# GenkiK/monodepth2

Measured on AMD Instinct MI355X. Metric: training images/sec at 640x192 mono, 1/2/4/8 GPUs; loss delta vs ref, higher is better.
Workload: dtype f32; 1 GPU; mono_640x192 ResNet-18 batch=12/GPU full train step (configs[1]); global_batch=12, height=192, width=640, parallelism=dp1, step=hipgraph replay

## Files before the change

### include/md2hot.h

```cpp
#ifndef MD2HOT_H
#define MD2HOT_H

#include <stddef.h>
#include <stdint.h>

#ifdef __cplusplus
extern "C" {
#endif

#define MD2_ABI_VERSION 24
#define MD2_MAX_SCALES 4
#define MD2_MAX_SRC 3

#define MD2_OK 0
#define MD2_ERR_ARG (-1)
#define MD2_ERR_HIP (-2)

#define MD2_NO_SSIM          (1u << 0)
#define MD2_AVG_REPROJECTION (1u << 1)
#define MD2_NO_AUTOMASK      (1u << 2)
#define MD2_V1_MULTISCALE    (1u << 3)
#define MD2_T_PER_SCALE      (1u << 4)
#define MD2_PREDICTIVE_MASK  (1u << 5)

// ... 66 lines not shown
size_t md2_decoder_pad_workspace_bytes(const md2_pad_desc* desc);
int md2_decoder_pad_fwd(const md2_pad_desc* desc, const float* x, const float* skip, const float* bias,
                        float* out, void* stream);
int md2_decoder_pad_bwd(const md2_pad_desc* desc, const float* x, const float* bias, const float* grad_out,
                        float* grad_x, float* grad_skip, float* grad_bias, void* workspace, void* stream);
int md2_decoder_pad_bwd2(const md2_pad_desc* desc, const float* x, const float* bias, const float* grad_out,
                         const float* grad_out2, float* grad_x, float* grad_skip, float* grad_bias, void* workspace,
                         void* stream);

#define MD2_HEAD_WEIGHT_CL (1u << 0)
#define MD2_HEAD_BF16 (1u << 1)

typedef struct md2_head_desc {
    int32_t batch, channels, height, width;
    uint32_t flags;
} md2_head_desc;

size_t md2_disp_head_workspace_bytes(const md2_head_desc* desc);
int md2_disp_head_fwd(const md2_head_desc* desc, const float* padded, const float* weight, const float* bias,
                      float* disp, void* stream);
int md2_disp_head_bwd(const md2_head_desc* desc, const float* padded, const float* weight, const float* disp,
                      const float* grad_disp, float* grad_padded, float* grad_weight, float* grad_bias,
                      void* workspace, void* stream);

#define MD2_STEM_WEIGHT_CL (1u << 0)
#define MD2_STEM_BF16 (1u << 1)
#define MD2_STEM_PREFETCH (1u << 2)

typedef struct md2_stem_desc {
    int32_t batch, channels, height, width;
    uint32_t flags;
} md2_stem_desc;

size_t md2_stem_wgrad_workspace_bytes(const md2_stem_desc* desc);
int md2_stem_wgrad(const md2_stem_desc* desc, const float* x, const float* grad_y, float* grad_weight,
                   void* workspace, void* stream);

int md2_stem_fwd(const md2_stem_desc* desc, const float* x, const float* weight, float* y, void* stream);

#define MD2_BIAS_ACT_RELU (1u << 0)

typedef struct md2_bias_act_desc {
    int64_t pixels;
    int32_t channels;
    uint32_t flags;
} md2_bias_act_desc;
// ... 266 lines not shown
```

### monodepth2_amd/_lib.py

```python
from __future__ import annotations

import ctypes
import os
import threading

import torch

from .build import LIB_PATH as _BUILT_LIB
from .build import source_hash

LIB_PATH = os.environ.get("MD2_LIB", _BUILT_LIB)

MAX_SCALES = 4
MAX_SRC = 3
ABI_VERSION = 24

NO_SSIM = 1 << 0
AVG_REPROJECTION = 1 << 1
NO_AUTOMASK = 1 << 2
V1_MULTISCALE = 1 << 3
T_PER_SCALE = 1 << 4
PREDICTIVE_MASK = 1 << 5

_vp = ctypes.c_void_p
# ... 23 lines not shown
_lib = None

EXPORTS = ["md2_abi_version", "md2_last_error", "md2_workspace_bytes", "md2_select_bytes",
           "md2_photometric_fwd", "md2_photometric_bwd", "md2_generate_images", "md2_tiebreak_noise",
           "md2_timing_begin", "md2_timing_end", "md2_timing_calls", "md2_decoder_pad_fwd", "md2_decoder_pad_bwd",
           "md2_decoder_pad_workspace_bytes", "md2_adam_step", "md2_adam_step_dev", "md2_adam_hyper", "md2_adam_apply_dev", "md2_encoder_input",
           "md2_pose_fwd", "md2_pose_bwd", "md2_aug_plan_create", "md2_aug_plan_destroy", "md2_aug_run",
           "md2_bn_workspace_bytes", "md2_bn_fwd", "md2_bn_bwd", "md2_maxpool3s2_fwd", "md2_maxpool3s2_bwd",
           "md2_disp_head_workspace_bytes", "md2_disp_head_fwd", "md2_disp_head_bwd",
           "md2_stem_wgrad_workspace_bytes", "md2_stem_wgrad", "md2_stem_fwd", "md2_conv_col2im", "md2_bias_act_fwd", "md2_bias_act_bwd",
           "md2_bias_act_workspace_bytes", "md2_maxpool3s2_bwd_add", "md2_bn_bwd_multi",
           "md2_conv_fwd", "md2_conv_workspace_bytes", "md2_conv_split_weights",
           "md2_conv_dgrad", "md2_conv_wgrad", "md2_conv_direct", "md2_conv_wgrad_direct",
           "md2_conv_wgrad_direct_workspace_bytes", "md2_conv_split_weights_multi", "md2_bn_fwd_mask",
           "md2_bn_bwd_mask", "md2_build_id", "md2_maxpool3s2_bwd_multi", "md2_decoder_pad_bwd2", "md2_aug_run2",
           "md2_conv_bf16_weights", "md2_conv_bf16_weights_multi",
           "md2_depth_eval", "md2_depth_eval_workspace_bytes",
           "md2_velo_project", "md2_velo_project_workspace_bytes",
           "md2_pose_ate", "md2_pose_ate_workspace_bytes",
           "md2_disp_colorize", "md2_disp_colorize_workspace_bytes",
           "md2_bn_pool_fwd_supported", "md2_bn_pool_fwd", "md2_bn_bwd_reduce_mask", "md2_bn_coef_offset",
           "md2_stem_wgrad_bn_supported", "md2_stem_wgrad_bn",
           "md2_aug_plan_create_mixed", "md2_aug_run_mixed",
           "md2_depth_export16", "md2_depth_export16_check"]

DTYPE_F32 = 0
DTYPE_BF16 = 1
PAD_ELU = 1 << 0
PAD_UPSAMPLE = 1 << 1
PAD_NHWC = 1 << 2
PAD_BF16 = 1 << 3


class PadDesc(ctypes.Structure):
    _fields_ = [("batch", ctypes.c_int32), ("channels", ctypes.c_int32), ("height", ctypes.c_int32),
                ("width", ctypes.c_int32), ("skip_channels", ctypes.c_int32), ("flags", ctypes.c_uint32)]


class AugDesc(ctypes.Structure):
    _fields_ = [("items", ctypes.c_int32), ("frames", ctypes.c_int32), ("in_height", ctypes.c_int32),
                ("in_width", ctypes.c_int32), ("height", ctypes.c_int32), ("width", ctypes.c_int32),
                ("num_scales", ctypes.c_int32), ("reserved", ctypes.c_int32)]


class AugItem(ctypes.Structure):
    _fields_ = [("flip", ctypes.c_uint8), ("color_aug", ctypes.c_uint8), ("hue_shift", ctypes.c_uint8),
                ("reserved", ctypes.c_uint8), ("order", ctypes.c_uint8 * 4), ("brightness", ctypes.c_float),
# ... 173 lines not shown
    L.md2_conv_split_weights.argtypes = [ctypes.POINTER(ConvDesc)] + [_vp] * 4
    L.md2_conv_split_weights_multi.restype = ctypes.c_int
    L.md2_conv_split_weights_multi.argtypes = [_vp, ctypes.c_int, ctypes.c_int, _vp]
    L.md2_conv_bf16_weights.restype = ctypes.c_int
    L.md2_conv_bf16_weights.argtypes = [ctypes.POINTER(ConvDesc)] + [_vp] * 4
    L.md2_conv_bf16_weights_multi.restype = ctypes.c_int
    L.md2_conv_bf16_weights_multi.argtypes = [_vp, ctypes.c_int, ctypes.c_int, _vp]
    L.md2_conv_workspace_bytes.restype = ctypes.c_size_t
    L.md2_conv_workspace_bytes.argtypes = [ctypes.POINTER(ConvDesc)]
    L.md2_stem_wgrad_workspace_bytes.restype = ctypes.c_size_t
    L.md2_stem_wgrad_workspace_bytes.argtypes = [ctypes.POINTER(StemDesc)]
    L.md2_stem_wgrad.restype = ctypes.c_int
    L.md2_stem_wgrad.argtypes = [ctypes.POINTER(StemDesc)] + [_vp] * 5
    L.md2_stem_fwd.restype = ctypes.c_int
    L.md2_conv_col2im.restype = ctypes.c_int
    L.md2_conv_col2im.argtypes = [ctypes.POINTER(ConvDesc)] + [_vp] * 3
    L.md2_stem_fwd.argtypes = [ctypes.POINTER(StemDesc)] + [_vp] * 4
    L.md2_disp_head_workspace_bytes.restype = ctypes.c_size_t
    L.md2_disp_head_workspace_bytes.argtypes = [ctypes.POINTER(HeadDesc)]
    L.md2_disp_head_fwd.restype = ctypes.c_int
    L.md2_disp_head_fwd.argtypes = [ctypes.POINTER(HeadDesc)] + [_vp] * 5
    L.md2_disp_head_bwd.restype = ctypes.c_int
    L.md2_disp_head_bwd.argtypes = [ctypes.POINTER(HeadDesc)] + [_vp] * 9
    L.md2_abi_version.restype = ctypes.c_int
    L.md2_abi_version.argtypes = []
    L.md2_build_id.restype = ctypes.c_char_p
    L.md2_build_id.argtypes = []
    L.md2_last_error.restype = ctypes.c_char_p
    L.md2_last_error.argtypes = []
    L.md2_workspace_bytes.restype = ctypes.c_size_t
    L.md2_workspace_bytes.argtypes = [ctypes.POINTER(Desc)]
    L.md2_select_bytes.restype = ctypes.c_size_t
    L.md2_select_bytes.argtypes = [ctypes.POINTER(Desc)]
    L.md2_photometric_fwd.restype = ctypes.c_int
    L.md2_photometric_fwd.argtypes = [ctypes.POINTER(Desc), ctypes.POINTER(Tensors), _vp, _vp, _vp, _vp]
    L.md2_photometric_bwd.restype = ctypes.c_int
    L.md2_photometric_bwd.argtypes = [ctypes.POINTER(Desc), ctypes.POINTER(Tensors), _vp, _vp,
                                      ctypes.POINTER(_vp), _vp, _vp, _vp, _vp]
    L.md2_generate_images.restype = ctypes.c_int
    L.md2_generate_images.argtypes = [ctypes.POINTER(Desc), ctypes.POINTER(Tensors),
                                      ctypes.POINTER(_vp), ctypes.POINTER(_vp), ctypes.POINTER(_vp), _vp]
    L.md2_tiebreak_noise.restype = ctypes.c_int
    L.md2_tiebreak_noise.argtypes = [ctypes.POINTER(Desc), _vp, ctypes.c_int, _vp, _vp]
    L.md2_decoder_pad_fwd.restype = ctypes.c_int
    L.md2_decoder_pad_fwd.argtypes = [ctypes.POINTER(PadDesc), _vp, _vp, _vp, _vp, _vp]
    L.md2_decoder_pad_bwd.restype = ctypes.c_int
# ... 125 lines not shown
```

### monodepth2_amd/build.py

```python
from __future__ import annotations

import hashlib
import os
import shutil
import subprocess
import sys

HERE = os.path.dirname(os.path.abspath(__file__))
CSRC = os.path.join(HERE, "csrc")
INCLUDE = os.path.join(os.path.dirname(HERE), "include")
LIB_NAME = "libmd2hot.so"
LIB_PATH = os.path.join(CSRC, LIB_NAME)
SOURCES = ["md2hot.hip", "decoder.hip", "pose.hip", "augment.hip", "bnorm.hip", "pool.hip", "adam.hip", "disphead.hip", "stem.hip", "bias_act.hip", "conv.hip", "direct.hip", "glue.hip", "eval.hip", "velo.hip", "traj.hip", "viz.hip"]
HEADERS = [os.path.join(INCLUDE, "md2hot.h"), os.path.join(CSRC, "md2_bf16.h"), os.path.join(CSRC, "md2_bn_expr.h"),
           os.path.join(CSRC, "md2_x6.h")]
ARCH = os.environ.get("MD2_OFFLOAD_ARCH", "gfx950")


def hipcc() -> str:
    for cand in (os.environ.get("HIPCC"), "/opt/rocm/bin/hipcc", shutil.which("hipcc")):
        if cand and os.path.exists(cand):
            return cand
    raise RuntimeError("hipcc not found (ROCm toolchain required to build libmd2hot.so)")


def needs_build() -> bool:
    if not os.path.exists(LIB_PATH):
        return True
    t = os.path.getmtime(LIB_PATH)
    deps = [os.path.join(CSRC, s) for s in SOURCES] + HEADERS
    if any(os.path.getmtime(d) > t for d in deps):
        return True
    return built_id(LIB_PATH) != source_hash()


def built_id(path: str):
    try:
        with open(path, "rb") as f:
# ... 62 lines not shown
```

### monodepth2_amd/csrc/decoder.hip

```cpp

#include <hip/hip_runtime.h>

#include <stdint.h>
#include <stdlib.h>

#include "md2_bf16.h"
#include "md2hot.h"

namespace {

constexpr int kThreads = 256;

__device__ __forceinline__ int reflect1(int i, int n) {
    return i < 0 ? -i : (i >= n ? 2 * n - 2 - i : i);
}

__device__ __forceinline__ float elu(float v) { return v > 0.f ? v : expm1f(v); }
__device__ __forceinline__ float elu_grad(float v) { return v > 0.f ? 1.f : expm1f(v) + 1.f; }

struct PadArgs {
    int B, C, Cs, h, w, H, W;
    const float* x;
    const float* skip;
    float* out;
    const float* gout;
    const float* gout2;
    float* gx;
    float* gskip;
    const float* bias;
    float* gbias_part;
};

template <bool NHWC>
__device__ __forceinline__ size_t at(int b, int c, int y, int x, int C, int Hh, int Ww) {
    return NHWC ? (((size_t)b * Hh + y) * Ww + x) * C + c : (((size_t)b * C + c) * Hh + y) * Ww + x;
}

template <bool ELU, bool UP, bool NHWC>
__global__ __launch_bounds__(kThreads) void pad_fwd_kernel(PadArgs a) {
    const int Hp = a.H + 2, Wp = a.W + 2, Ct = a.C + a.Cs;
    const long long total = (long long)a.B * Ct * Hp * Wp;
    for (long long idx = (long long)blockIdx.x * kThreads + threadIdx.x; idx < total;
         idx += (long long)gridDim.x * kThreads) {
        int px, py, c, b;
        long long t;
        if (NHWC) {
            c = (int)(idx % Ct);
            t = idx / Ct;
            px = (int)(t % Wp);
            t /= Wp;
            py = (int)(t % Hp);
            b = (int)(t / Hp);
        } else {
// ... 66 lines not shown
        int b, c, i, j;
        if (idx < nx) {
            coords<NHWC>(idx, a.C, a.h, a.w, b, c, i, j);
            const float* g = a.gout + at<NHWC>(b, c, 0, 0, Ct, Hp, Wp);
            float s;
            if (UP) {
                s = fold(g, Wp, a.H, a.W, 2 * i, 2 * j, es) + fold(g, Wp, a.H, a.W, 2 * i, 2 * j + 1, es) +
                    fold(g, Wp, a.H, a.W, 2 * i + 1, 2 * j, es) + fold(g, Wp, a.H, a.W, 2 * i + 1, 2 * j + 1, es);
            } else {
                s = fold(g, Wp, a.H, a.W, i, j, es);
            }
            if (ELU) s *= elu_grad(a.x[idx]);
            a.gx[idx] = s;
        } else {
            const long long k = idx - nx;
            coords<NHWC>(k, a.Cs, a.H, a.W, b, c, i, j);
            a.gskip[k] = fold(a.gout + at<NHWC>(b, a.C + c, 0, 0, Ct, Hp, Wp), Wp, a.H, a.W, i, j, es);
        }
    }
}

__device__ __forceinline__ float4 ld4(const float* p) { return *(const float4*)p; }
__device__ __forceinline__ void st4(float* p, float4 v) { *(float4*)p = v; }
__device__ __forceinline__ float4 add4(float4 a, float4 b) { return {a.x + b.x, a.y + b.y, a.z + b.z, a.w + b.w}; }

template <typename T, bool ELU, bool UP>
__global__ __launch_bounds__(kThreads) void pad_fwd_v4_kernel(PadArgs a) {
    const int Hp = a.H + 2, Wp = a.W + 2, Ct4 = (a.C + a.Cs) / 4;
    const int total = a.B * Hp * Wp * Ct4;
    for (int idx = blockIdx.x * kThreads + threadIdx.x; idx < total; idx += gridDim.x * kThreads) {
        const int c = 4 * (idx % Ct4);
        int t = idx / Ct4;
        const int px = t % Wp;
        t /= Wp;
        const int py = t % Hp;
        const int b = t / Hp;
        const int yy = reflect1(py - 1, a.H), xx = reflect1(px - 1, a.W);
        float4 v;
        if (c < a.C) {
            const int sy = UP ? (yy >> 1) : yy, sx = UP ? (xx >> 1) : xx;
            v = md2::ld4T<T>(a.x, (((size_t)b * a.h + sy) * a.w + sx) * a.C + c);
            if (a.bias) v = add4(v, ld4(a.bias + c));
            if (ELU) v = {elu(v.x), elu(v.y), elu(v.z), elu(v.w)};
        } else {
            v = md2::ld4T<T>(a.skip, (((size_t)b * a.H + yy) * a.W + xx) * a.Cs + (c - a.C));
        }
        md2::st4T<T>(a.out, 4 * (size_t)idx, v);
    }
}

template <typename T>
__device__ __forceinline__ float4 fold4(const float* gout, const float* gout2, size_t g0, int Wp, int H, int W,
                                        int yy, int xx, int Ct) {
    auto G = [&](int y, int x) {
        const size_t o = g0 + ((size_t)y * Wp + x) * Ct;
        float4 v = md2::ld4T<T>(gout, o);
        if (gout2) v = add4(v, md2::ld4T<T>(gout2, o));
        return v;
    };
    float4 s = G(yy + 1, xx + 1);
    const bool ry = (yy == 1), ry2 = (yy == H - 2), rx = (xx == 1), rx2 = (xx == W - 2);
    if (rx) s = add4(s, G(yy + 1, 0));
    if (rx2) s = add4(s, G(yy + 1, W + 1));
    if (ry) {
        s = add4(s, G(0, xx + 1));
        if (rx) s = add4(s, G(0, 0));
        if (rx2) s = add4(s, G(0, W + 1));
    }
    if (ry2) {
        s = add4(s, G(H + 1, xx + 1));
        if (rx) s = add4(s, G(H + 1, 0));
        if (rx2) s = add4(s, G(H + 1, W + 1));
    }
    return s;
}

template <typename T, bool ELU, bool UP>
__global__ __launch_bounds__(kThreads) void pad_bwd_v4_kernel(PadArgs a) {
    const int Hp = a.H + 2, Wp = a.W + 2, Ct = a.C + a.Cs, C4 = a.C / 4, Cs4 = a.Cs / 4;
    const int nx = a.B * a.h * a.w * C4;
    const int ns = a.B * a.H * a.W * Cs4;
    float4 bsum = {0.f, 0.f, 0.f, 0.f};
    const float4 bq = a.bias ? ld4(a.bias + 4 * (threadIdx.x % C4)) : float4{0.f, 0.f, 0.f, 0.f};
    for (int idx = blockIdx.x * kThreads + threadIdx.x; idx < nx + ns; idx += gridDim.x * kThreads) {
        if (idx < nx) {
            const int c = 4 * (idx % C4);
            int t = idx / C4;
            const int j = t % a.w;
            t /= a.w;
            const int i = t % a.h;
            const int b = t / a.h;
            const size_t g = (size_t)b * Hp * Wp * Ct + c;
            float4 s;
            if (UP) {
                s = add4(add4(fold4<T>(a.gout, a.gout2, g, Wp, a.H, a.W, 2 * i, 2 * j, Ct),
                              fold4<T>(a.gout, a.gout2, g, Wp, a.H, a.W, 2 * i, 2 * j + 1, Ct)),
                         add4(fold4<T>(a.gout, a.gout2, g, Wp, a.H, a.W, 2 * i + 1, 2 * j, Ct),
                              fold4<T>(a.gout, a.gout2, g, Wp, a.H, a.W, 2 * i + 1, 2 * j + 1, Ct)));
            } else {
                s = fold4<T>(a.gout, a.gout2, g, Wp, a.H, a.W, i, j, Ct);
            }
            if (ELU) {
                float4 xv = md2::ld4T<T>(a.x, 4 * (size_t)idx);
                if (a.bias) xv = add4(xv, bq);
                s = {s.x * elu_grad(xv.x), s.y * elu_grad(xv.y), s.z * elu_grad(xv.z), s.w * elu_grad(xv.w)};
            }
            md2::st4T<T>(a.gx, 4 * (size_t)idx, s);
            bsum = add4(bsum, s);
        } else {
            const int k = idx - nx;
            const int c = 4 * (k % Cs4);
            int t = k / Cs4;
            const int xx = t % a.W;
            t /= a.W;
            const int yy = t % a.H;
            const int b = t / a.H;
            md2::st4T<T>(a.gskip, 4 * (size_t)k, fold4<T>(a.gout, a.gout2, (size_t)b * Hp * Wp * Ct + a.C + c, Wp, a.H, a.W, yy, xx, Ct));
        }
    }
    if (!a.gbias_part) return;
    __shared__ float4 red[kThreads];
// ... 325 lines not shown
    a.gbias_part = grad_bias ? (float*)workspace : nullptr;
    const long long n = (long long)a.B * a.C * a.h * a.w + (long long)a.B * a.Cs * a.H * a.W;
    if (vec8(d)) {
        const int G = grid_for(n / 8);
        hipLaunchKernelGGL(v8_bwd(elu, up), dim3(G), dim3(kThreads), 0, (hipStream_t)stream, a);
        if (grad_bias)
            hipLaunchKernelGGL(bias_grad_kernel, dim3(a.C), dim3(kThreads), 0, (hipStream_t)stream,
                               (const float*)workspace, G, grad_bias);
        return hipGetLastError() == hipSuccess ? MD2_OK : MD2_ERR_HIP;
    }
    if (vec4(d)) {
        PadFn k = (d->flags & MD2_PAD_BF16) ? v4_bwd<uint16_t>(elu, up) : v4_bwd<float>(elu, up);
        const int G = grid_for(n / 4);
        hipLaunchKernelGGL(k, dim3(G), dim3(kThreads), 0, (hipStream_t)stream, a);
        if (grad_bias)
            hipLaunchKernelGGL(bias_grad_kernel, dim3(a.C), dim3(kThreads), 0, (hipStream_t)stream,
                               (const float*)workspace, G, grad_bias);
        return hipGetLastError() == hipSuccess ? MD2_OK : MD2_ERR_HIP;
    }
    hipLaunchKernelGGL(bwd_kernel(d->flags), dim3(grid_for(n)), dim3(kThreads), 0, (hipStream_t)stream, a);
    return hipGetLastError() == hipSuccess ? MD2_OK : MD2_ERR_HIP;
}

}
```

### monodepth2_amd/csrc/disphead.hip

```cpp

#include <hip/hip_runtime.h>

#include <stdint.h>
#include <stdlib.h>

#include "md2_bf16.h"
#include "md2hot.h"

namespace {

constexpr int kThreads = 256;
constexpr int kMaxC = 256;
constexpr int kBwdBlocks = 2048;
constexpr int kFwdBlocks = 4096;
constexpr int kMaxLds = 64 * 1024;

struct HeadArgs {
    int B, C, h, w;
    int w_cl;
    const float* P;
    const float* wt;
    const float* bias;
    float* disp;
    const float* gdisp;
    float* gP;
    float* part;
    float* gw;
    float* gb;
};

__device__ __forceinline__ float4 wt_quad(const HeadArgs& a, int tap, int q) {
    if (a.w_cl) return reinterpret_cast<const float4*>(a.wt + tap * a.C)[q];
    const int c = q * 4;
    return make_float4(a.wt[c * 9 + tap], a.wt[(c + 1) * 9 + tap], a.wt[(c + 2) * 9 + tap], a.wt[(c + 3) * 9 + tap]);
}

__device__ __forceinline__ float dot4(float4 u, float4 v) { return u.x * v.x + u.y * v.y + u.z * v.z + u.w * v.w; }

template <bool BF>
__device__ __forceinline__ float4 ld_quad(const float* P, unsigned i) {
    if constexpr (BF) {
        const uint2 u = reinterpret_cast<const uint2*>(P)[i];
        return make_float4(md2::bf2f(u.x & 0xffffu), md2::bf2f(u.x >> 16), md2::bf2f(u.y & 0xffffu),
                           md2::bf2f(u.y >> 16));
    } else {
        return reinterpret_cast<const float4*>(P)[i];
    }
}
template <bool BF>
__device__ __forceinline__ void st_quad(float* G, unsigned i, float4 g) {
    if constexpr (BF)
        reinterpret_cast<uint2*>(G)[i] =
            make_uint2(md2::f2bf(g.x) | (md2::f2bf(g.y) << 16), md2::f2bf(g.z) | (md2::f2bf(g.w) << 16));
    else
        reinterpret_cast<float4*>(G)[i] = g;
}

// ... 76 lines not shown
        const int Y = y0 + r < Hp ? y0 + r : Hp - 1;
        const unsigned base = ((unsigned)(b * Hp + Y) * Wp + x) * Q + sub;
#pragma unroll
        for (int kx = 0; kx < 3; ++kx)
#pragma unroll
            for (int k = 0; k < QL; ++k) v[r][kx][k] = ld_quad<BF>(a.P, base + kx * Q + k * L);
    }
#pragma unroll
    for (int r = 0; r < R; ++r) {
        if (y0 + r >= a.h) break;
        float acc = 0.f;
#pragma unroll
        for (int ky = 0; ky < 3; ++ky)
#pragma unroll
            for (int kx = 0; kx < 3; ++kx)
#pragma unroll
                for (int k = 0; k < QL; ++k) acc += dot4(v[r + ky][kx][k], wr[ky * 3 + kx][k]);
#pragma unroll
        for (int o = L / 2; o > 0; o >>= 1) acc += __shfl_xor(acc, o, L);
        if (sub == 0) a.disp[((unsigned)b * a.h + y0 + r) * a.w + x] = 1.f / (1.f + expf(-(acc + bias)));
    }
}

template <int Q, bool BF = false>
__global__ __launch_bounds__(kThreads) void head_bwd_kernel(HeadArgs a) {
    extern __shared__ float lds[];
    constexpr int TP = kThreads / Q;
    const int Wp = a.w + 2, Hp = a.h + 2;
    const int Ws = Wp + 2;
    const int q = threadIdx.x % Q, p0 = threadIdx.x / Q;
    float4 wq[9];
#pragma unroll
    for (int tap = 0; tap < 9; ++tap) wq[tap] = wt_quad(a, tap, q);
    float4 dw[9];
#pragma unroll
    for (int tap = 0; tap < 9; ++tap) dw[tap] = make_float4(0.f, 0.f, 0.f, 0.f);
    float db = 0.f;
    const int rows = a.B * Hp;
    for (int r = blockIdx.x; r < rows; r += gridDim.x) {
        const int b = r / Hp, Y = r - b * Hp;
        __syncthreads();
        for (int e = threadIdx.x; e < 3 * Ws; e += kThreads) {
            const int ky = e / Ws, x = e - ky * Ws - 2, y = Y - ky;
            float dz = 0.f;
            if (y >= 0 && y < a.h && x >= 0 && x < a.w) {
                const int o = (b * a.h + y) * a.w + x;
                const float d = a.disp[o];
                dz = a.gdisp[o] * d * (1.f - d);
            }
            lds[e] = dz;
        }
        __syncthreads();
        const int rowbase = r * Wp;
        for (int X = p0; X < Wp; X += TP) {
            const int i = (rowbase + X) * Q + q;
            const float4 p = ld_quad<BF>(a.P, i);
            float4 g = make_float4(0.f, 0.f, 0.f, 0.f);
#pragma unroll
            for (int ky = 0; ky < 3; ++ky)
#pragma unroll
                for (int kx = 0; kx < 3; ++kx) {
                    const float dz = lds[ky * Ws + X + 2 - kx];
                    const int tap = ky * 3 + kx;
                    g.x += wq[tap].x * dz;
                    g.y += wq[tap].y * dz;
                    g.z += wq[tap].z * dz;
                    g.w += wq[tap].w * dz;
                    dw[tap].x += p.x * dz;
                    dw[tap].y += p.y * dz;
                    dw[tap].z += p.z * dz;
                    dw[tap].w += p.w * dz;
                }
            if (q == 0) db += lds[Ws + X + 1];
            st_quad<BF>(a.gP, i, g);
        }
    }
    float v[37];
#pragma unroll
    for (int tap = 0; tap < 9; ++tap) {
        v[tap * 4 + 0] = dw[tap].x;
        v[tap * 4 + 1] = dw[tap].y;
        v[tap * 4 + 2] = dw[tap].z;
        v[tap * 4 + 3] = dw[tap].w;
    }
    v[36] = db;
#pragma unroll
    for (int o = Q; o < 64; o <<= 1)
#pragma unroll
        for (int j = 0; j < 37; ++j) v[j] += __shfl_xor(v[j], o, 64);
    const int lane = threadIdx.x % 64, wave = threadIdx.x / 64;
    __syncthreads();
    if (lane < Q) {
        float* dst = lds + (wave * Q + lane) * 37;
#pragma unroll
        for (int j = 0; j < 37; ++j) dst[j] = v[j];
    }
    __syncthreads();
// ... 131 lines not shown
    a.P = padded;
    a.wt = weight;
    a.disp = const_cast<float*>(disp);
    a.gdisp = grad_disp;
    a.gP = grad_padded;
    a.part = (float*)workspace;
    a.gw = grad_weight;
    a.gb = grad_bias;
    const int G = bwd_grid(a);
    const int Q = a.C / 4;
    const bool bf = (d->flags & MD2_HEAD_BF16) != 0;
    void (*k)(HeadArgs) = Q == 1    ? (bf ? head_bwd_kernel<1, true> : head_bwd_kernel<1>)
                          : Q == 2  ? (bf ? head_bwd_kernel<2, true> : head_bwd_kernel<2>)
                          : Q == 4  ? (bf ? head_bwd_kernel<4, true> : head_bwd_kernel<4>)
                          : Q == 8  ? (bf ? head_bwd_kernel<8, true> : head_bwd_kernel<8>)
                          : Q == 16 ? (bf ? head_bwd_kernel<16, true> : head_bwd_kernel<16>)
                          : Q == 32 ? (bf ? head_bwd_kernel<32, true> : head_bwd_kernel<32>)
                                    : (bf ? head_bwd_kernel<64, true> : head_bwd_kernel<64>);
    hipLaunchKernelGGL(k, dim3(G), dim3(kThreads), bwd_lds(a.C, a.w), (hipStream_t)stream, a);
    hipLaunchKernelGGL(head_wgrad_kernel, dim3(9 * a.C + 1), dim3(kThreads), 0, (hipStream_t)stream, a, G);
    return hipGetLastError() == hipSuccess ? MD2_OK : MD2_ERR_HIP;
}

}
```

### monodepth2_amd/decoder_ops.py

```python
from __future__ import annotations

import ctypes
import os
from typing import Optional

import torch
import torch.nn.functional as F

from . import _lib


_CL = torch.channels_last


def _flags(elu: bool, upsample: bool, nhwc: bool, bf16: bool = False) -> int:
    return ((_lib.PAD_ELU if elu else 0) | (_lib.PAD_UPSAMPLE if upsample else 0) | (_lib.PAD_NHWC if nhwc else 0)
            | (_lib.PAD_BF16 if bf16 else 0))


class _ConvInput(torch.autograd.Function):

    @staticmethod
    def forward(ctx, x, skip, bias, elu: bool, upsample: bool, nhwc: bool, alias: bool = False):
        fmt = _CL if nhwc else torch.contiguous_format
# ... 91 lines not shown
                         device=P.device)
        rc = _lib.lib().md2_disp_head_bwd(ctypes.byref(d), P.data_ptr(), weight.data_ptr(), disp.data_ptr(),
                                          gdisp.data_ptr(), gP.data_ptr(), gw.data_ptr(), gb.data_ptr(),
                                          ws.data_ptr(), _lib.stream(P.device))
        _lib.check(rc, "md2_disp_head_bwd")
        return gP, gw, gb


def supports_disp_head(P: torch.Tensor, conv: torch.nn.Conv2d, bf16_input: bool = False) -> bool:
    C = P.shape[1]
    want = torch.bfloat16 if bf16_input else torch.float32
    return (P.is_cuda and P.dtype == want and conv.weight.dtype == torch.float32
            and P.is_contiguous(memory_format=_CL) and conv.out_channels == 1 and conv.bias is not None
            and tuple(conv.kernel_size) == (3, 3) and tuple(conv.padding) == (0, 0)
            and tuple(conv.stride) == (1, 1) and C % 4 == 0 and C <= 256 and 256 % (C // 4) == 0)


def disp_head(P: torch.Tensor, conv: torch.nn.Conv2d) -> torch.Tensor:
    if not supports_disp_head(P, conv, bf16_input=P.dtype == torch.bfloat16):
        raise ValueError("disp_head: fp32 / bf16 channels_last input, Conv2d(C, 1, 3) with bias, C/4 dividing 256")
    return _DispHead.apply(P, conv.weight, conv.bias)


_POSE_MIOPEN = os.environ.get("MD2_POSE_MIOPEN", "0") == "1"


class _BiasAct(torch.autograd.Function):

    @staticmethod
    def forward(ctx, z, bias, relu: bool):
        B, C, H, W = z.shape
        d = _lib.BiasActDesc(B * H * W, C, _lib.BIAS_ACT_RELU if relu else 0)
        _lib.check(_lib.lib().md2_bias_act_fwd(ctypes.byref(d), z.data_ptr(), bias.data_ptr(), z.data_ptr(),
                                               _lib.stream(z.device)),
                   "md2_bias_act_fwd")
        ctx.mark_dirty(z)
        ctx.save_for_backward(z if relu else None)
        ctx.conf = (relu, d)
        return z

    @staticmethod
    def backward(ctx, gy):
        y, = ctx.saved_tensors
        relu, d = ctx.conf
        gy = gy.contiguous(memory_format=_CL)
        gb = torch.empty(gy.shape[1], device=gy.device, dtype=torch.float32)
# ... 96 lines not shown
```

### monodepth2_amd/networks/decoders.py

```python
from __future__ import annotations

import numpy as np
import torch
import torch.nn as nn
import torch.nn.functional as F

from ..layers import Conv3x3, ConvBlock, upsample

import os

_AMP_HEADS = os.environ.get("MD2_AMP_FUSED_HEADS", "1") != "0"


class DepthDecoder(nn.Module):

    def __init__(self, num_ch_enc, scales=range(4), num_output_channels=1, use_skips=True):
        super().__init__()
        self.num_output_channels = num_output_channels
        self.use_skips = use_skips
        self.upsample_mode = "nearest"
        self.scales = scales
        self.num_ch_enc = num_ch_enc
        self.num_ch_dec = np.array([16, 32, 64, 128, 256])
        ch_enc, ch_dec = self.num_ch_enc, self.num_ch_dec
        self.convs = {}
        mods = []
        for i in range(4, -1, -1):
            cin = ch_enc[-1] if i == 4 else ch_dec[i + 1]
            self.convs[("upconv", i, 0)] = ConvBlock(cin, ch_dec[i])
            cin = ch_dec[i] + (ch_enc[i - 1] if (use_skips and i > 0) else 0)
            self.convs[("upconv", i, 1)] = ConvBlock(cin, ch_dec[i])
            mods += [self.convs[("upconv", i, 0)], self.convs[("upconv", i, 1)]]
        for s in self.scales:
            self.convs[("dispconv", s)] = Conv3x3(ch_dec[s], num_output_channels)
            mods.append(self.convs[("dispconv", s)])
        self.decoder = nn.ModuleList(mods)
        self.sigmoid = nn.Sigmoid()
        self.fused = True
        self.fused_heads = True

    def _forward_fused(self, input_features):
        from ..conv_ops import conv2d_w
        from ..decoder_ops import conv_input, disp_head, supports_bias, supports_disp_head
        self.outputs = {}
        cl = self.convs[("upconv", 4, 0)].conv.conv.weight.is_contiguous(memory_format=torch.channels_last)
        P = conv_input(input_features[-1], nhwc=cl)

        def conv(block, P):
            c = block.conv.conv
            if c.bias is not None and supports_bias(c.out_channels, cl) and c.groups == 1 \
                    and tuple(c.dilation) == (1, 1) and c.stride[0] == c.stride[1] and c.padding[0] == c.padding[1]:
                return conv2d_w(P, c.weight, c.stride[0], c.padding[0]), c.bias
            return c(P), None

        for i in range(4, -1, -1):
            y0, b0 = conv(self.convs[("upconv", i, 0)], P)
            skip = input_features[i - 1] if (self.use_skips and i > 0) else None
            P = conv_input(y0, skip, elu=True, upsample=True, nhwc=cl, bias=b0)
            y1, b1 = conv(self.convs[("upconv", i, 1)], P)
            if i in self.scales and i > 0:
                P, Ph = conv_input(y1, None, elu=True, upsample=False, nhwc=cl, bias=b1, alias=True)
            else:
                P = Ph = conv_input(y1, None, elu=True, upsample=False, nhwc=cl, bias=b1)
            if i in self.scales:
                head = self.convs[("dispconv", i)].conv
                if self.fused_heads and supports_disp_head(Ph, head) and not torch.is_autocast_enabled():
                    self.outputs[("disp", i)] = disp_head(Ph, head)
                elif (self.fused_heads and _AMP_HEADS and torch.is_autocast_enabled()
                        and supports_disp_head(Ph, head, bf16_input=True)):
                    with torch.autocast("cuda", enabled=False):
                        self.outputs[("disp", i)] = disp_head(Ph, head)
                else:
                    self.outputs[("disp", i)] = self.sigmoid(head(Ph))
        return self.outputs

    def forward(self, input_features):
        f = input_features[-1]
        cl = self.convs[("upconv", 4, 0)].conv.conv.weight.is_contiguous(memory_format=torch.channels_last)
        if (f.is_cuda and self.fused and self.num_output_channels >= 1
                and (f.dtype == torch.float32 or (f.dtype == torch.bfloat16 and cl))):
            return self._forward_fused(input_features)
        self.outputs = {}
# ... 64 lines not shown
```

Baseline: 1133 images/s.

## Fuse scale-0 bias+ELU+reflect-pad into disparity head forward and backward

At the full-resolution decoder scale, the disparity head now reads the pre-activation conv output and its bias directly. It applies bias+ELU and reflection padding on the fly inside a tiled forward kernel, so the padded activation tensor is never written. In backward, the head kernel can skip writing the padded-input gradient and emit only dz. The pad-backward kernel then recomputes the head's input gradient from dz and the 3x3 weights using DPP quad broadcasts, avoiding a large 16-channel gradient round-trip through memory at the cost of extra arithmetic and more complex kernels.

Result: no change. 1137 images/s, median of 6 (+0.3%).

```diff
diff --git a/include/md2hot.h b/include/md2hot.h
--- a/include/md2hot.h
+++ b/include/md2hot.h
@@ -112,6 +112,14 @@
 int md2_disp_head_bwd(const md2_head_desc* desc, const float* padded, const float* weight, const float* disp,
                       const float* grad_disp, float* grad_padded, float* grad_weight, float* grad_bias,
                       void* workspace, void* stream);
+int md2_disp_head_src_fwd(const md2_head_desc* desc, const float* src, const float* src_bias, const float* weight,
+                          const float* bias, float* disp, void* stream);
+int md2_disp_head_src_bwd(const md2_head_desc* desc, const float* src, const float* src_bias, const float* weight,
+                          const float* disp, const float* grad_disp, float* grad_padded, float* head_dz,
+                          float* grad_weight, float* grad_bias, void* workspace, void* stream);
+int md2_decoder_pad_bwd_head(const md2_pad_desc* desc, const float* x, const float* bias, const float* head_dz,
+                             const float* head_weight, int head_weight_cl, float* grad_x, float* grad_bias,
+                             void* workspace, void* stream);
 
 #define MD2_STEM_WEIGHT_CL (1u << 0)
 #define MD2_STEM_BF16 (1u << 1)
diff --git a/monodepth2_amd/_lib.py b/monodepth2_amd/_lib.py
--- a/monodepth2_amd/_lib.py
+++ b/monodepth2_amd/_lib.py
@@ -69,7 +69,8 @@
            "md2_bn_pool_fwd_supported", "md2_bn_pool_fwd", "md2_bn_bwd_reduce_mask", "md2_bn_coef_offset",
            "md2_stem_wgrad_bn_supported", "md2_stem_wgrad_bn",
            "md2_aug_plan_create_mixed", "md2_aug_run_mixed",
-           "md2_depth_export16", "md2_depth_export16_check"]
+           "md2_depth_export16", "md2_depth_export16_check",
+           "md2_disp_head_src_fwd", "md2_disp_head_src_bwd", "md2_decoder_pad_bwd_head"]
 
 DTYPE_F32 = 0
 DTYPE_BF16 = 1
@@ -289,6 +290,12 @@
     L.md2_disp_head_fwd.argtypes = [ctypes.POINTER(HeadDesc)] + [_vp] * 5
     L.md2_disp_head_bwd.restype = ctypes.c_int
     L.md2_disp_head_bwd.argtypes = [ctypes.POINTER(HeadDesc)] + [_vp] * 9
+    L.md2_disp_head_src_fwd.restype = ctypes.c_int
+    L.md2_disp_head_src_fwd.argtypes = [ctypes.POINTER(HeadDesc)] + [_vp] * 6
+    L.md2_disp_head_src_bwd.restype = ctypes.c_int
+    L.md2_disp_head_src_bwd.argtypes = [ctypes.POINTER(HeadDesc)] + [_vp] * 11
+    L.md2_decoder_pad_bwd_head.restype = ctypes.c_int
+    L.md2_decoder_pad_bwd_head.argtypes = [ctypes.POINTER(PadDesc), _vp, _vp, _vp, _vp, ctypes.c_int, _vp, _vp, _vp, _vp]
     L.md2_abi_version.restype = ctypes.c_int
     L.md2_abi_version.argtypes = []
     L.md2_build_id.restype = ctypes.c_char_p
diff --git a/monodepth2_amd/build.py b/monodepth2_amd/build.py
--- a/monodepth2_amd/build.py
+++ b/monodepth2_amd/build.py
@@ -13,7 +13,7 @@
 LIB_PATH = os.path.join(CSRC, LIB_NAME)
 SOURCES = ["md2hot.hip", "decoder.hip", "pose.hip", "augment.hip", "bnorm.hip", "pool.hip", "adam.hip", "disphead.hip", "stem.hip", "bias_act.hip", "conv.hip", "direct.hip", "glue.hip", "eval.hip", "velo.hip", "traj.hip", "viz.hip"]
 HEADERS = [os.path.join(INCLUDE, "md2hot.h"), os.path.join(CSRC, "md2_bf16.h"), os.path.join(CSRC, "md2_bn_expr.h"),
-           os.path.join(CSRC, "md2_x6.h")]
+           os.path.join(CSRC, "md2_x6.h"), os.path.join(CSRC, "md2_dec_expr.h")]
 ARCH = os.environ.get("MD2_OFFLOAD_ARCH", "gfx950")
 
 
diff --git a/monodepth2_amd/csrc/decoder.hip b/monodepth2_amd/csrc/decoder.hip
--- a/monodepth2_amd/csrc/decoder.hip
+++ b/monodepth2_amd/csrc/decoder.hip
@@ -5,18 +5,17 @@
 #include <stdlib.h>
 
 #include "md2_bf16.h"
+#include "md2_dec_expr.h"
 #include "md2hot.h"
 
 namespace {
 
 constexpr int kThreads = 256;
 
-__device__ __forceinline__ int reflect1(int i, int n) {
-    return i < 0 ? -i : (i >= n ? 2 * n - 2 - i : i);
-}
-
-__device__ __forceinline__ float elu(float v) { return v > 0.f ? v : expm1f(v); }
-__device__ __forceinline__ float elu_grad(float v) { return v > 0.f ? 1.f : expm1f(v) + 1.f; }
+using md2::add4;
+using md2::elu;
+using md2::elu_grad;
+using md2::reflect1;
 
 struct PadArgs {
     int B, C, Cs, h, w, H, W;
@@ -29,6 +28,9 @@
     float* gskip;
     const float* bias;
     float* gbias_part;
+    const float* hdz;
+    const float* hwt;
+    int hw_cl;
 };
 
 template <bool NHWC>
@@ -141,7 +143,6 @@
 
 __device__ __forceinline__ float4 ld4(const float* p) { return *(const float4*)p; }
 __device__ __forceinline__ void st4(float* p, float4 v) { *(float4*)p = v; }
-__device__ __forceinline__ float4 add4(float4 a, float4 b) { return {a.x + b.x, a.y + b.y, a.z + b.z, a.w + b.w}; }
 
 template <typename T, bool ELU, bool UP>
 __global__ __launch_bounds__(kThreads) void pad_fwd_v4_kernel(PadArgs a) {
@@ -177,30 +178,31 @@
         if (gout2) v = add4(v, md2::ld4T<T>(gout2, o));
         return v;
     };
-    float4 s = G(yy + 1, xx + 1);
-    const bool ry = (yy == 1), ry2 = (yy == H - 2), rx = (xx == 1), rx2 = (xx == W - 2);
-    if (rx) s = add4(s, G(yy + 1, 0));
-    if (rx2) s = add4(s, G(yy + 1, W + 1));
-    if (ry) {
-        s = add4(s, G(0, xx + 1));
-        if (rx) s = add4(s, G(0, 0));
-        if (rx2) s = add4(s, G(0, W + 1));
-    }
-    if (ry2) {
-        s = add4(s, G(H + 1, xx + 1));
-        if (rx) s = add4(s, G(H + 1, 0));
-        if (rx2) s = add4(s, G(H + 1, W + 1));
-    }
-    return s;
-}
-
-template <typename T, bool ELU, bool UP>
+    return md2::fold4(G, H, W, yy, xx);
+}
+
+__device__ __forceinline__ float quad_bcast(float v, int k) {
+    const int i = __float_as_int(v);
+    const int r = k == 0   ? __builtin_amdgcn_update_dpp(0, i, 0x00, 0xf, 0xf, false)
+                  : k == 1 ? __builtin_amdgcn_update_dpp(0, i, 0x55, 0xf, 0xf, false)
+                  : k == 2 ? __builtin_amdgcn_update_dpp(0, i, 0xaa, 0xf, 0xf, false)
+                           : __builtin_amdgcn_update_dpp(0, i, 0xff, 0xf, 0xf, false);
+    return __int_as_float(r);
+}
+
+template <typename T, bool ELU, bool UP, bool HEADG = false>
 __global__ __launch_bounds__(kThreads) void pad_bwd_v4_kernel(PadArgs a) {
     const int Hp = a.H + 2, Wp = a.W + 2, Ct = a.C + a.Cs, C4 = a.C / 4, Cs4 = a.Cs / 4;
     const int nx = a.B * a.h * a.w * C4;
     const int ns = a.B * a.H * a.W * Cs4;
     float4 bsum = {0.f, 0.f, 0.f, 0.f};
     const float4 bq = a.bias ? ld4(a.bias + 4 * (threadIdx.x % C4)) : float4{0.f, 0.f, 0.f, 0.f};
+    __shared__ float4 hw[HEADG ? 9 : 1][4];
+    if constexpr (HEADG) {
+        if (threadIdx.x < 36) hw[threadIdx.x >> 2][threadIdx.x & 3] =
+            md2::head_wt_quad(a.hwt, a.C, a.hw_cl, threadIdx.x >> 2, threadIdx.x & 3);
+        __syncthreads();
+    }
     for (int idx = blockIdx.x * kThreads + threadIdx.x; idx < nx + ns; idx += gridDim.x * kThreads) {
         if (idx < nx) {
             const int c = 4 * (idx % C4);
@@ -216,6 +218,27 @@
                               fold4<T>(a.gout, a.gout2, g, Wp, a.H, a.W, 2 * i, 2 * j + 1, Ct)),
                          add4(fold4<T>(a.gout, a.gout2, g, Wp, a.H, a.W, 2 * i + 1, 2 * j, Ct),
                               fold4<T>(a.gout, a.gout2, g, Wp, a.H, a.W, 2 * i + 1, 2 * j + 1, Ct)));
+            } else if constexpr (HEADG) {
+                const float* dzb = a.hdz + (size_t)b * a.H * a.W;
+                const int ql = threadIdx.x & 3;
+                auto G = [&](int Y, int X) {
+                    float r[3];
+                    const int y = Y - ql;
+#pragma unroll
+                    for (int kx = 0; kx < 3; ++kx) {
+                        const int x = X - kx;
+                        const bool in = ql < 3 && (unsigned)y < (unsigned)a.H && (unsigned)x < (unsigned)a.W;
+                        r[kx] = in ? dzb[y * a.W + x] : 0.f;
+                    }
+                    float4 gq = make_float4(0.f, 0.f, 0.f, 0.f);
+#pragma unroll
+                    for (int ky = 0; ky < 3; ++ky)
+#pragma unroll
+                        for (int kx = 0; kx < 3; ++kx)
+                            md2::head_tap_g(gq, hw[ky * 3 + kx][ql], quad_bcast(r[kx], ky));
+                    return gq;
+                };
+                s = md2::fold4_rolled(G, a.H, a.W, i, j);
             } else {
                 s = fold4<T>(a.gout, a.gout2, g, Wp, a.H, a.W, i, j, Ct);
             }
@@ -587,4 +610,29 @@
     return hipGetLastError() == hipSuccess ? MD2_OK : MD2_ERR_HIP;
 }
 
-}
+int md2_decoder_pad_bwd_head(const md2_pad_desc* d, const float* x, const float* bias, const float* head_dz,
+                             const float* head_weight, int head_weight_cl, float* grad_x, float* grad_bias,
+                             void* workspace, void* stream) {
+    PadArgs a = {};
+    if (!make_args(d, a) || d->flags != (MD2_PAD_ELU | MD2_PAD_NHWC) || a.C != 16 || a.Cs != 0 || !x || !head_dz ||
+        !head_weight || !grad_x)
+        return MD2_ERR_ARG;
+    if (grad_bias && (!bias || !workspace)) return MD2_ERR_ARG;
+    a.x = x;
+    a.gx = grad_x;
+    a.bias = bias;
+    a.gbias_part = grad_bias ? (float*)workspace : nullptr;
+    a.hdz = head_dz;
+    a.hwt = head_weight;
+    a.hw_cl = head_weight_cl ? 1 : 0;
+    const long long n = (long long)a.B * a.C * a.h * a.w;
+    const int G = grid_for(n / 4);
+    hipLaunchKernelGGL((pad_bwd_v4_kernel<float, true, false, true>), dim3(G), dim3(kThreads), 0, (hipStream_t)stream,
+                       a);
+    if (grad_bias)
+        hipLaunchKernelGGL(bias_grad_kernel, dim3(a.C), dim3(kThreads), 0, (hipStream_t)stream,
+                           (const float*)workspace, G, grad_bias);
+    return hipGetLastError() == hipSuccess ? MD2_OK : MD2_ERR_HIP;
+}
+
+}
diff --git a/monodepth2_amd/csrc/disphead.hip b/monodepth2_amd/csrc/disphead.hip
--- a/monodepth2_amd/csrc/disphead.hip
+++ b/monodepth2_amd/csrc/disphead.hip
@@ -5,6 +5,7 @@
 #include <stdlib.h>
 
 #include "md2_bf16.h"
+#include "md2_dec_expr.h"
 #include "md2hot.h"
 
 namespace {
@@ -27,12 +28,18 @@
     float* part;
     float* gw;
     float* gb;
+    const float* sbias;
+    float* dzout;
 };
 
 __device__ __forceinline__ float4 wt_quad(const HeadArgs& a, int tap, int q) {
-    if (a.w_cl) return reinterpret_cast<const float4*>(a.wt + tap * a.C)[q];
-    const int c = q * 4;
-    return make_float4(a.wt[c * 9 + tap], a.wt[(c + 1) * 9 + tap], a.wt[(c + 2) * 9 + tap], a.wt[(c + 3) * 9 + tap]);
+    return md2::head_wt_quad(a.wt, a.C, a.w_cl, tap, q);
+}
+
+__device__ __forceinline__ float4 src_quad(const HeadArgs& a, int b, int Y, int X, int Q, int q, float4 bq) {
+    const int yy = md2::pad_src<false>(Y, a.h), xx = md2::pad_src<false>(X, a.w);
+    const float4 v = reinterpret_cast<const float4*>(a.P)[((unsigned)(b * a.h + yy) * a.w + xx) * Q + q];
+    return md2::bias_elu4(v, bq);
 }
 
 __device__ __forceinline__ float dot4(float4 u, float4 v) { return u.x * v.x + u.y * v.y + u.z * v.z + u.w * v.w; }
@@ -155,7 +162,57 @@
     }
 }
 
-template <int Q, bool BF = false>
+__global__ __launch_bounds__(kThreads) void head_fwd_src_kernel(HeadArgs a) {
+    constexpr int L = 4, Q = 4, GPB = kThreads / L, R = 8, NR = R + 2, NC = GPB + 2;
+    __shared__ float4 tile[NR][NC][Q];
+    const int Wp = a.w + 2, Hp = a.h + 2;
+    const int sub = threadIdx.x % L, grp = threadIdx.x / L;
+    const int ntx = (a.w + GPB - 1) / GPB, nty = (a.h + R - 1) / R;
+    int t = blockIdx.x;
+    const int tx = t % ntx;
+    t /= ntx;
+    const int ty = t % nty, b = t / nty;
+    const int x = tx * GPB + grp, y0 = ty * R;
+    float4 wr[9];
+#pragma unroll
+    for (int tap = 0; tap < 9; ++tap) wr[tap] = wt_quad(a, tap, sub);
+    const float bias = a.bias[0];
+    const float4 bq = reinterpret_cast<const float4*>(a.sbias)[sub];
+    if (x + 1 < Wp) {
+#pragma unroll
+        for (int r = 0; r < NR; ++r) {
+            const int Y = y0 + r < Hp ? y0 + r : Hp - 1;
+            tile[r][grp + 1][sub] = src_quad(a, b, Y, x + 1, Q, sub, bq);
+        }
+    }
+    if ((int)threadIdx.x < 2 * NR * Q) {
+        const int side = threadIdx.x / (NR * Q), r = threadIdx.x % (NR * Q) / Q, q = threadIdx.x % Q;
+        const int c = side * (GPB + 1), X = tx * GPB + c;
+        const int Y = y0 + r < Hp ? y0 + r : Hp - 1;
+        if (X < Wp) tile[r][c][q] = src_quad(a, b, Y, X, Q, q, reinterpret_cast<const float4*>(a.sbias)[q]);
+    }
+    __syncthreads();
+    if (x >= a.w) return;
+    float4 v[NR][3];
+#pragma unroll
+    for (int r = 0; r < NR; ++r)
+#pragma unroll
+        for (int kx = 0; kx < 3; ++kx) v[r][kx] = tile[r][grp + kx][sub];
+#pragma unroll
+    for (int r = 0; r < R; ++r) {
+        if (y0 + r >= a.h) break;
+        float acc = 0.f;
+#pragma unroll
+        for (int ky = 0; ky < 3; ++ky)
+#pragma unroll
+            for (int kx = 0; kx < 3; ++kx) acc += dot4(v[r + ky][kx], wr[ky * 3 + kx]);
+#pragma unroll
+        for (int o = L / 2; o > 0; o >>= 1) acc += __shfl_xor(acc, o, L);
+        if (sub == 0) a.disp[((unsigned)b * a.h + y0 + r) * a.w + x] = 1.f / (1.f + expf(-(acc + bias)));
+    }
+}
+
+template <int Q, bool BF = false, bool SRC = false, bool NOGP = false>
 __global__ __launch_bounds__(kThreads) void head_bwd_kernel(HeadArgs a) {
     extern __shared__ float lds[];
     constexpr int TP = kThreads / Q;
@@ -169,6 +226,8 @@
 #pragma unroll
     for (int tap = 0; tap < 9; ++tap) dw[tap] = make_float4(0.f, 0.f, 0.f, 0.f);
     float db = 0.f;
+    float4 bq = make_float4(0.f, 0.f, 0.f, 0.f);
+    if constexpr (SRC) bq = reinterpret_cast<const float4*>(a.sbias)[q];
     const int rows = a.B * Hp;
     for (int r = blockIdx.x; r < rows; r += gridDim.x) {
         const int b = r / Hp, Y = r - b * Hp;
@@ -178,8 +237,10 @@
             float dz = 0.f;
             if (y >= 0 && y < a.h && x >= 0 && x < a.w) {
                 const int o = (b * a.h + y) * a.w + x;
-                const float d = a.disp[o];
-                dz = a.gdisp[o] * d * (1.f - d);
+                dz = md2::head_dz(a.gdisp[o], a.disp[o]);
+                if constexpr (NOGP) {
+                    if (ky == 0) a.dzout[o] = dz;
+                }
             }
             lds[e] = dz;
         }
@@ -187,7 +248,9 @@
         const int rowbase = r * Wp;
         for (int X = p0; X < Wp; X += TP) {
             const int i = (rowbase + X) * Q + q;
-            const float4 p = ld_quad<BF>(a.P, i);
+            float4 p;
+            if constexpr (SRC) p = src_quad(a, b, Y, X, Q, q, bq);
+            else p = ld_quad<BF>(a.P, i);
             float4 g = make_float4(0.f, 0.f, 0.f, 0.f);
 #pragma unroll
             for (int ky = 0; ky < 3; ++ky)
@@ -195,17 +258,11 @@
                 for (int kx = 0; kx < 3; ++kx) {
                     const float dz = lds[ky * Ws + X + 2 - kx];
                     const int tap = ky * 3 + kx;
-                    g.x += wq[tap].x * dz;
-                    g.y += wq[tap].y * dz;
-                    g.z += wq[tap].z * dz;
-                    g.w += wq[tap].w * dz;
-                    dw[tap].x += p.x * dz;
-                    dw[tap].y += p.y * dz;
-                    dw[tap].z += p.z * dz;
-                    dw[tap].w += p.w * dz;
+                    if constexpr (!NOGP) md2::head_tap_g(g, wq[tap], dz);
+                    md2::head_tap_dw(dw[tap], p, dz);
                 }
             if (q == 0) db += lds[Ws + X + 1];
-            st_quad<BF>(a.gP, i, g);
+            if constexpr (!NOGP) st_quad<BF>(a.gP, i, g);
         }
     }
     float v[37];
@@ -383,4 +440,48 @@
     return hipGetLastError() == hipSuccess ? MD2_OK : MD2_ERR_HIP;
 }
 
-}
+static bool valid_src(const md2_head_desc* d) {
+    return valid(d) && d->channels == 16 && !(d->flags & MD2_HEAD_BF16) && d->height >= 2 && d->width >= 2;
+}
+
+int md2_disp_head_src_fwd(const md2_head_desc* d, const float* src, const float* src_bias, const float* weight,
+                          const float* bias, float* disp, void* stream) {
+    if (!valid_src(d) || !src || !src_bias || !weight || !bias || !disp) return MD2_ERR_ARG;
+    HeadArgs a = args_of(d);
+    a.P = src;
+    a.sbias = src_bias;
+    a.wt = weight;
+    a.bias = bias;
+    a.disp = disp;
+    constexpr int L = 4, R = 8, GPB = kThreads / L;
+    const long long tiles = (long long)((a.w + GPB - 1) / GPB) * ((a.h + R - 1) / R) * a.B;
+    if (tiles >= (1ll << 31)) return MD2_ERR_ARG;
+    hipLaunchKernelGGL(head_fwd_src_kernel, dim3((unsigned)tiles), dim3(kThreads), 0, (hipStream_t)stream, a);
+    return hipGetLastError() == hipSuccess ? MD2_OK : MD2_ERR_HIP;
+}
+
+int md2_disp_head_src_bwd(const md2_head_desc* d, const float* src, const float* src_bias, const float* weight,
+                          const float* disp, const float* grad_disp, float* grad_padded, float* head_dz,
+                          float* grad_weight, float* grad_bias, void* workspace, void* stream) {
+    if (!valid_src(d) || !src || !src_bias || !weight || !disp || !grad_disp || (!grad_padded == !head_dz) ||
+        !grad_weight || !grad_bias || !workspace)
+        return MD2_ERR_ARG;
+    HeadArgs a = args_of(d);
+    a.P = src;
+    a.sbias = src_bias;
+    a.wt = weight;
+    a.disp = const_cast<float*>(disp);
+    a.gdisp = grad_disp;
+    a.gP = grad_padded;
+    a.dzout = head_dz;
+    a.part = (float*)workspace;
+    a.gw = grad_weight;
+    a.gb = grad_bias;
+    const int G = bwd_grid(a);
+    void (*k)(HeadArgs) = grad_padded ? head_bwd_kernel<4, false, true, false> : head_bwd_kernel<4, false, true, true>;
+    hipLaunchKernelGGL(k, dim3(G), dim3(kThreads), bwd_lds(a.C, a.w), (hipStream_t)stream, a);
+    hipLaunchKernelGGL(head_wgrad_kernel, dim3(9 * a.C + 1), dim3(kThreads), 0, (hipStream_t)stream, a, G);
+    return hipGetLastError() == hipSuccess ? MD2_OK : MD2_ERR_HIP;
+}
+
+}
diff --git a/monodepth2_amd/csrc/md2_dec_expr.h b/monodepth2_amd/csrc/md2_dec_expr.h
--- /dev/null
+++ b/monodepth2_amd/csrc/md2_dec_expr.h
@@ -0,0 +1,76 @@
+#pragma once
+
+#include <hip/hip_runtime.h>
+
+namespace md2 {
+
+__device__ __forceinline__ int reflect1(int i, int n) {
+    return i < 0 ? -i : (i >= n ? 2 * n - 2 - i : i);
+}
+template <bool UP>
+__device__ __forceinline__ int pad_src(int p, int n) {
+    const int r = reflect1(p - 1, n);
+    return UP ? (r >> 1) : r;
+}
+
+__device__ __forceinline__ float elu(float v) { return v > 0.f ? v : expm1f(v); }
+__device__ __forceinline__ float elu_grad(float v) { return v > 0.f ? 1.f : expm1f(v) + 1.f; }
+
+__device__ __forceinline__ float4 add4(float4 a, float4 b) { return {a.x + b.x, a.y + b.y, a.z + b.z, a.w + b.w}; }
+__device__ __forceinline__ float4 elu4(float4 v) { return {elu(v.x), elu(v.y), elu(v.z), elu(v.w)}; }
+__device__ __forceinline__ float4 bias_elu4(float4 v, float4 b) { return elu4(add4(v, b)); }
+
+template <typename GF>
+__device__ __forceinline__ float4 fold4(GF G, int H, int W, int yy, int xx) {
+    float4 s = G(yy + 1, xx + 1);
+    const bool ry = (yy == 1), ry2 = (yy == H - 2), rx = (xx == 1), rx2 = (xx == W - 2);
+    if (rx) s = add4(s, G(yy + 1, 0));
+    if (rx2) s = add4(s, G(yy + 1, W + 1));
+    if (ry) {
+        s = add4(s, G(0, xx + 1));
+        if (rx) s = add4(s, G(0, 0));
+        if (rx2) s = add4(s, G(0, W + 1));
+    }
+    if (ry2) {
+        s = add4(s, G(H + 1, xx + 1));
+        if (rx) s = add4(s, G(H + 1, 0));
+        if (rx2) s = add4(s, G(H + 1, W + 1));
+    }
+    return s;
+}
+
+template <typename GF>
+__device__ __forceinline__ float4 fold4_rolled(GF G, int H, int W, int yy, int xx) {
+    const bool ry = (yy == 1), ry2 = (yy == H - 2), rx = (xx == 1), rx2 = (xx == W - 2);
+    const int nr = 1 + ry + ry2, nc = 1 + rx + rx2;
+    float4 s = G(yy + 1, xx + 1);
+#pragma unroll 1
+    for (int k = 1; k < nr * nc; ++k) {
+        const int a = k / nc, c = k - a * nc;
+        const int y = a == 0 ? yy + 1 : ((a == 1 && ry) ? 0 : H + 1);
+        const int x = c == 0 ? xx + 1 : ((c == 1 && rx) ? 0 : W + 1);
+        s = add4(s, G(y, x));
+    }
+    return s;
+}
+
+__device__ __forceinline__ float4 head_wt_quad(const float* wt, int C, int w_cl, int tap, int q) {
+    if (w_cl) return reinterpret_cast<const float4*>(wt + tap * C)[q];
+    const int c = q * 4;
+    return make_float4(wt[c * 9 + tap], wt[(c + 1) * 9 + tap], wt[(c + 2) * 9 + tap], wt[(c + 3) * 9 + tap]);
+}
+__device__ __forceinline__ float head_dz(float gd, float d) { return gd * d * (1.f - d); }
+__device__ __forceinline__ void head_tap_g(float4& g, const float4 w, const float dz) {
+    g.x = __builtin_fmaf(w.x, dz, g.x);
+    g.y = __builtin_fmaf(w.y, dz, g.y);
+    g.z = __builtin_fmaf(w.z, dz, g.z);
+    g.w = __builtin_fmaf(w.w, dz, g.w);
+}
+__device__ __forceinline__ void head_tap_dw(float4& dw, const float4 p, const float dz) {
+    dw.x = __builtin_fmaf(p.x, dz, dw.x);
+    dw.y = __builtin_fmaf(p.y, dz, dw.y);
+    dw.z = __builtin_fmaf(p.z, dz, dw.z);
+    dw.w = __builtin_fmaf(p.w, dz, dw.w);
+}
+
+}
diff --git a/monodepth2_amd/decoder_ops.py b/monodepth2_amd/decoder_ops.py
--- a/monodepth2_amd/decoder_ops.py
+++ b/monodepth2_amd/decoder_ops.py
@@ -137,6 +137,86 @@
     return _DispHead.apply(P, conv.weight, conv.bias)
 
 
+DEC_FUSE = os.environ.get("MD2_DEC_FUSE", "1") != "0"
+DEC_FUSE_HEAD = os.environ.get("MD2_DEC_FUSE_HEAD", "1") != "0"
+DEC_FUSE_HEADBWD = os.environ.get("MD2_DEC_FUSE_HEADBWD", "1") != "0"
+
+
+def _pad_bwd2(d, x, bias32, gout, gx, gbias):
+    L = _lib.lib()
+    ws = torch.empty(L.md2_decoder_pad_workspace_bytes(ctypes.byref(d)), dtype=torch.uint8, device=x.device)
+    _lib.check(L.md2_decoder_pad_bwd2(ctypes.byref(d), x.data_ptr(), bias32.data_ptr(), gout.data_ptr(), None,
+                                      gx.data_ptr(), None, gbias.data_ptr(), ws.data_ptr(), _lib.stream(x.device)),
+               "md2_decoder_pad_bwd2")
+
+
+class _DispHeadSrc(torch.autograd.Function):
+
+    @staticmethod
+    def forward(ctx, y1, b1, weight, bias, no_gp: bool):
+        y1 = y1.contiguous(memory_format=_CL)
+        B, C, h, w = y1.shape
+        w_cl = weight.is_contiguous(memory_format=_CL)
+        if not w_cl:
+            weight = weight.contiguous()
+        b32 = b1.detach().contiguous()
+        d = _lib.HeadDesc(B, C, h, w, _lib.HEAD_WEIGHT_CL if w_cl else 0)
+        disp = torch.empty(B, 1, h, w, device=y1.device, dtype=torch.float32)
+        _lib.check(_lib.lib().md2_disp_head_src_fwd(ctypes.byref(d), y1.data_ptr(), b32.data_ptr(), weight.data_ptr(),
+                                                    bias.data_ptr(), disp.data_ptr(), _lib.stream(y1.device)),
+                   "md2_disp_head_src_fwd")
+        ctx.d, ctx.w_cl, ctx.no_gp = d, w_cl, no_gp
+        ctx.save_for_backward(y1, b32, weight, disp)
+        return disp
+
+    @staticmethod
+    def backward(ctx, gdisp):
+        y1, b32, weight, disp = ctx.saved_tensors
+        d = ctx.d
+        B, C, h, w = y1.shape
+        dev = y1.device
+        L = _lib.lib()
+        gdisp = gdisp.float().contiguous()
+        gw = torch.empty_like(weight)
+        gb = torch.empty(1, device=dev, dtype=torch.float32)
+        ws = torch.empty(L.md2_disp_head_workspace_bytes(ctypes.byref(d)), dtype=torch.uint8, device=dev)
+        gy1 = torch.empty_like(y1, memory_format=_CL)
+        gb1 = torch.empty(C, device=dev, dtype=torch.float32)
+        pd = _lib.PadDesc(B, C, h, w, 0, _flags(True, False, True))
+        if ctx.no_gp:
+            dz = torch.empty(B, h, w, device=dev, dtype=torch.float32)
+            gP = None
+        else:
+            dz = None
+            gP = torch.empty(B, C, h + 2, w + 2, device=dev, dtype=torch.float32, memory_format=_CL)
+        _lib.check(L.md2_disp_head_src_bwd(ctypes.byref(d), y1.data_ptr(), b32.data_ptr(), weight.data_ptr(),
+                                           disp.data_ptr(), gdisp.data_ptr(),
+                                           gP.data_ptr() if gP is not None else None,
+                                           dz.data_ptr() if dz is not None else None, gw.data_ptr(), gb.data_ptr(),
+                                           ws.data_ptr(), _lib.stream(dev)), "md2_disp_head_src_bwd")
+        if ctx.no_gp:
+            pws = torch.empty(L.md2_decoder_pad_workspace_bytes(ctypes.byref(pd)), dtype=torch.uint8, device=dev)
+            _lib.check(L.md2_decoder_pad_bwd_head(ctypes.byref(pd), y1.data_ptr(), b32.data_ptr(), dz.data_ptr(),
+                                                  weight.data_ptr(), 1 if ctx.w_cl else 0, gy1.data_ptr(),
+                                                  gb1.data_ptr(), pws.data_ptr(), _lib.stream(dev)),
+                       "md2_decoder_pad_bwd_head")
+        else:
+            _pad_bwd2(pd, y1, b32, gP, gy1, gb1)
+        return gy1, gb1, gw, gb, None
+
+
+def supports_disp_head_src(y1: torch.Tensor, b1: Optional[torch.Tensor], conv: torch.nn.Conv2d) -> bool:
+    return (DEC_FUSE and DEC_FUSE_HEAD and b1 is not None and b1.dtype == torch.float32 and y1.dim() == 4
+            and y1.shape[1] == 16 and y1.shape[2] >= 2 and y1.shape[3] >= 2 and not torch.is_autocast_enabled()
+            and supports_disp_head(y1, conv))
+
+
+def disp_head_src(y1: torch.Tensor, b1: torch.Tensor, conv: torch.nn.Conv2d) -> torch.Tensor:
+    if not supports_disp_head_src(y1, b1, conv):
+        raise ValueError("disp_head_src: fp32 channels_last (B, 16, h >= 2, w >= 2) input with its conv's bias")
+    return _DispHeadSrc.apply(y1, b1, conv.weight, conv.bias, DEC_FUSE_HEADBWD)
+
+
 _POSE_MIOPEN = os.environ.get("MD2_POSE_MIOPEN", "0") == "1"
 
 
diff --git a/monodepth2_amd/networks/decoders.py b/monodepth2_amd/networks/decoders.py
--- a/monodepth2_amd/networks/decoders.py
+++ b/monodepth2_amd/networks/decoders.py
@@ -41,7 +41,8 @@
 
     def _forward_fused(self, input_features):
         from ..conv_ops import conv2d_w
-        from ..decoder_ops import conv_input, disp_head, supports_bias, supports_disp_head
+        from ..decoder_ops import (conv_input, disp_head, disp_head_src, supports_bias, supports_disp_head,
+                                   supports_disp_head_src)
         self.outputs = {}
         cl = self.convs[("upconv", 4, 0)].conv.conv.weight.is_contiguous(memory_format=torch.channels_last)
         P = conv_input(input_features[-1], nhwc=cl)
@@ -58,6 +59,10 @@
             skip = input_features[i - 1] if (self.use_skips and i > 0) else None
             P = conv_input(y0, skip, elu=True, upsample=True, nhwc=cl, bias=b0)
             y1, b1 = conv(self.convs[("upconv", i, 1)], P)
+            if (i == 0 and i in self.scales and cl and self.fused_heads
+                    and supports_disp_head_src(y1, b1, self.convs[("dispconv", i)].conv)):
+                self.outputs[("disp", i)] = disp_head_src(y1, b1, self.convs[("dispconv", i)].conv)
+                continue
             if i in self.scales and i > 0:
                 P, Ph = conv_input(y1, None, elu=True, upsample=False, nhwc=cl, bias=b1, alias=True)
             else:
```
